# jinlong17/DA-Detect

Measured on AMD Instinct MI355X. Metric: train images/sec, DA-Faster-RCNN R-50 Cityscapes->Foggy, higher is better.
Workload: dtype f32

## Files before the change

da_detect_amd/_C.py:

```python
import contextlib
import os
import ctypes
import time

import torch

from . import _lib
from . import amax as _amax
from ._lib import ConvDesc

CL = torch.channels_last

NMS_TIE_RULE = 0

PROFILER = None
_KNAME_CACHE = {}


class KernelProfiler(object):

    def __init__(self, pool=0, only=None):
        self.only = only
        self._pool = []
        for _ in range(pool):
# ... 328 lines not shown

def _transpose_now(w, scale, wt):
    Cout, Cin, KH, KW = w.shape
    cout_pad = wt.shape[1]
    _lib.call("dadet_conv_weight_transpose_padded", _p(w), _p(scale), _p(wt), Cout, KH, KW, Cin, cout_pad, _stream())
    return wt


class _TransposeCache(object):

    def __init__(self):
        self.entries = {}
        self.epoch = 0
        self.batched_epoch = -1
        self.table = None
        self.ready = None
        self.enabled = True
        self._from_bump = False
        self._trained_only = False

    def bump(self, device=None, trained_only=False):
        self.epoch += 1
        self._trained_only = bool(trained_only)
        if self.enabled and device is not None and self.entries:
            self._from_bump = True
            try:
                self._refresh_all(device)
            finally:
                self._from_bump = False
        elif device is not None and _mode4():
            _amax.WEIGHTS.refresh(device, self.epoch, trained_only=self._trained_only)
        self._trained_only = False

    def _single(self, e, w, scale):
        _transpose_now(w, scale, e["wt"])
        _amax.WEIGHTS.invalidate(e["wt"])
        e["epoch"] = self.epoch
        if w.is_cuda:
            st = torch.cuda.current_stream(w.device)
            e["ev"] = (st, st.record_event())
        return e["wt"]

    def get(self, w, scale, cout_pad=0):
        Cout, Cin, KH, KW = w.shape
        key = (w.data_ptr(), Cout, Cin, KH, KW, scale.data_ptr() if scale is not None else 0, w.device.index, cout_pad)
        e = self.entries.get(key)
        if e is None:
            wt = torch.empty((Cin, max(Cout, cout_pad), KH, KW), dtype=torch.float32, device=w.device, memory_format=CL)
            wt._dadet_persistent = True
            e = self.entries[key] = dict(w=w, scale=scale, wt=wt, version=w._version, epoch=self.epoch, used=self.epoch,
                                         ev=None)
            self.table = None
            return self._single(e, w, scale)
        e["used"] = self.epoch
        if e["version"] != w._version:
            e["w"], e["version"] = w, w._version
            return self._single(e, w, scale)
        if e["epoch"] != self.epoch:
            if self.batched_epoch != self.epoch:
                self._refresh_all(w.device)
            if e["epoch"] != self.epoch:
                return self._single(e, w, scale)
        src = e["ev"] if e["ev"] is not None else self.ready
        if src is not None and w.is_cuda and torch.cuda.current_stream(w.device) != src[0]:
            torch.cuda.current_stream(w.device).wait_event(src[1])
        return e["wt"]
# ... 957 lines not shown
```

da_detect_amd/_lib.py:

```python
import ctypes
import os
from ctypes import POINTER, c_char_p, c_float, c_int, c_int64, c_size_t, c_uint64, c_void_p

_HERE = os.path.dirname(os.path.abspath(__file__))
LIB_PATH = os.environ.get("DADET_LIB") or os.path.join(_HERE, "libdadet_hip.so")
_lib = None
DEFAULT_GEMM_MODE = "4"


class ConvDesc(ctypes.Structure):

    _fields_ = [(n, c_int) for n in (
        "N", "H", "W", "Cin", "Cout", "KH", "KW", "stride", "pad", "Ho", "Wo", "OutH", "OutW",
        "out_spatial_stride", "relu_mode")]


class WgradPending(ctypes.Structure):

    _fields_ = [("partials", c_void_p), ("out_scale", c_void_p), ("dw", c_void_p), ("count", ctypes.c_longlong),
                ("K", c_int), ("splits", c_int), ("accumulate", c_int)]


class TransposeItem(ctypes.Structure):
    _fields_ = [("w", c_void_p), ("scale", c_void_p), ("wt", c_void_p), ("Cout", c_int), ("KH", c_int), ("KW", c_int),
                ("Cin", c_int), ("first_block", c_int), ("blocks_ci", c_int), ("blocks_co", c_int), ("cout_pad", c_int)]


class AmaxItem(ctypes.Structure):

    _fields_ = [("x", c_void_p), ("slot", c_void_p), ("n", ctypes.c_longlong), ("first_block", c_int), ("blocks", c_int)]


class MergeEntry(ctypes.Structure):

    _fields_ = [("boxes", c_void_p), ("scores", c_void_p), ("keep", c_void_p), ("count", c_void_p), ("boxes_out", c_void_p),
                ("scores_out", c_void_p), ("n", c_int), ("cap", c_int)]


class TopkRow(ctypes.Structure):

    _fields_ = [("scores", c_void_p), ("out_scores", c_void_p), ("out_idx", c_void_p), ("n", c_int), ("k", c_int)]


class SgdEntry(ctypes.Structure):

    _fields_ = [("p", c_void_p), ("g", c_void_p), ("buf", c_void_p), ("numel", c_int64),
                ("lr", c_float), ("weight_decay", c_float)]


_P = c_void_p
_SIGNATURES = {
    "dadet_version": [],
    "dadet_device_info": [POINTER(c_int), POINTER(c_int), POINTER(c_size_t), c_char_p, c_int],
    "dadet_nms_workspace_bytes": [c_int, POINTER(c_size_t)],
    "dadet_nms": [_P, _P, c_int, c_float, c_int, c_int, _P, c_size_t, _P, _P, _P],
    "dadet_roi_align_forward": [_P, _P, _P, c_int, c_int, c_int, c_int, c_int, c_int, c_int, c_float, c_int, _P],
    "dadet_roi_align_backward": [_P, _P, _P, c_int, c_int, c_int, c_int, c_int, c_int, c_int, c_float, c_int, _P],
    "dadet_roi_align_workspace_bytes": [c_int, c_int, c_int, c_int, POINTER(c_size_t)],
    "dadet_roi_align_forward_ws": [_P, _P, _P, c_int, c_int, c_int, c_int, c_int, c_int, c_int, c_float, c_int, _P, c_size_t, _P],
    "dadet_roi_align_backward_atomic": [_P, _P, _P, c_int, c_int, c_int, c_int, c_int, c_int, c_int, c_float, c_int, _P],
    "dadet_roi_align_forward_sub": [_P, _P, _P, c_int, c_int, c_int, c_int, c_int, c_int, c_int, c_float, c_int, c_int,
                                    _P, c_size_t, _P],
    "dadet_roi_align_forward_level": [_P, _P, _P, c_int, _P, c_int, c_int, c_int, c_int, c_int, c_int, c_int, c_float, c_int, _P,
                                      c_size_t, _P],
    "dadet_roi_align_backward_level": [_P, _P, _P, c_int, _P, c_int, c_int, c_int, c_int, c_int, c_int, c_int, c_float, c_int,
                                       _P],
    "dadet_roi_align_backward_sub": [_P, _P, _P, c_int, c_int, c_int, c_int, c_int, c_int, c_int, c_float, c_int, c_int,
                                     _P],
    "dadet_sigmoid_focal_loss_forward": [_P, _P, _P, c_int, c_int, c_float, c_float, _P],
    "dadet_sigmoid_focal_loss_backward": [_P, _P, _P, _P, c_int, c_int, c_float, c_float, _P],
    "dadet_conv_forward": [POINTER(ConvDesc), _P, _P, _P, _P, _P, _P, _P, _P],
    "dadet_conv_forward_scaled": [POINTER(ConvDesc), _P, _P, _P, _P, _P, _P, _P, _P, _P, _P, _P],
    "dadet_conv_wgrad_scaled": [POINTER(ConvDesc), _P, _P, c_int, _P, _P, c_int, _P, c_size_t, POINTER(WgradPending), _P, _P,
                                _P],
    "dadet_amax": [_P, ctypes.c_longlong, _P, _P],
    "dadet_amax_batch": [_P, c_int, c_int, _P],
    "dadet_conv_forward_variant": [POINTER(ConvDesc)],
    "dadet_set_gemm_mode": [c_int],
    "dadet_get_gemm_mode": [],
    "dadet_conv_wgrad_variant": [POINTER(ConvDesc)],
# ... 46 lines not shown
    "dadet_rpn_anchor_targets": [_P, _P, c_int, _P, c_int, c_float, c_float, _P, _P, _P, _P],
    "dadet_box_match_encode": [_P, c_int, _P, _P, c_int, c_float, c_float, c_float, c_float, c_float, c_float, _P, _P,
                               _P, _P],
    "dadet_roi_pool_forward": [_P, _P, _P, _P, c_int, c_int, c_int, c_int, c_int, c_int, c_int, c_float, _P],
    "dadet_roi_pool_backward": [_P, _P, _P, _P, c_int, c_int, c_int, c_int, c_int, c_int, c_int, _P],
    "dadet_deform_psroi_pool_forward": [_P, _P, _P, _P, _P, c_int, c_int, c_int, c_int, c_int, c_int, c_float,
                                        c_int, c_int, c_int, c_int, c_int, c_float, c_int, _P],
    "dadet_deform_psroi_pool_backward": [_P, _P, _P, _P, _P, _P, _P, c_int, c_int, c_int, c_int, c_int, c_int,
                                         c_float, c_int, c_int, c_int, c_int, c_int, c_float, c_int, _P],
    "dadet_relu_bn_backward": [_P, _P, _P, _P, _P, c_int64, c_int, _P],
    "dadet_relu_bn_backward_m": [_P, _P, _P, _P, _P, c_int64, c_int, _P, _P, _P],
    "dadet_colsum_workspace_bytes": [c_int64, c_int, POINTER(c_size_t)],
    "dadet_colsum": [_P, _P, c_int64, c_int, _P, c_size_t, _P],
    "dadet_colsum_ld": [_P, c_int, _P, c_int64, c_int, c_int, _P, c_size_t, _P],
    "dadet_channel_affine": [_P, _P, _P, _P, c_int64, c_int, c_int, _P],
    "dadet_maxpool3x3s2_forward": [_P, _P, c_int, c_int, c_int, c_int, c_int, c_int, _P],
    "dadet_avgpool_forward": [_P, _P, c_int, c_int, c_int, _P],
    "dadet_avgpool_backward": [_P, _P, c_int, c_int, c_int, _P],
    "dadet_nchw3_to_nhwc4": [_P, _P, c_int, c_int, c_int, _P],
    "dadet_rpn_decode_clip": [_P, _P, _P, c_int, c_float, c_float, c_float, c_float, c_float, c_float, c_float, _P, _P],
    "dadet_da_img_head_loss_forward": [_P, _P, _P, _P, _P, _P, c_int, c_int, c_int, _P],
    "dadet_da_img_head_loss_backward": [_P, _P, _P, _P, _P, _P, _P, _P, _P, c_int, c_int, c_int, _P],
    "dadet_da_img_head_loss_backward_g": [_P, _P, _P, _P, _P, _P, _P, c_float, c_float, _P, _P, _P, _P, c_int, c_int, c_int,
                                          _P],
    "dadet_da_img_head_loss_backward_gm": [_P, _P, _P, _P, _P, _P, _P, c_float, c_float, _P, _P, _P, _P, c_int, c_int, c_int,
                                          _P, _P, _P],
    "dadet_da_ins_tail_forward": [_P, _P, _P, _P, _P, _P, _P, c_int, c_int, c_int, c_int, c_int, _P],
    "dadet_da_ins_tail_backward": [_P, _P, _P, _P, _P, _P, c_float, _P, _P, _P, _P, c_int, c_int, c_int, c_int, c_int, _P],
    "dadet_da_ins_dropout_rows": [_P, _P, _P, c_int64, c_int, _P],
    "dadet_da_ins_merge": [_P, _P, _P, _P, _P, _P, c_int64, c_int, _P],
    "dadet_triplet_w_forward": [_P, _P, _P, c_int, c_int, c_int, c_float, c_float, _P, _P, _P],
    "dadet_triplet_w_backward": [_P, _P, _P, _P, _P, c_int, c_int, c_int, c_float, c_float, _P, _P, _P, _P],
    "dadet_sgd_step": [_P, c_int, c_int64, c_float, c_int, c_float, _P],
}
_RESTYPES = {"dadet_last_error": c_char_p}
EXPORTED_SYMBOLS = sorted(list(_SIGNATURES) + ["dadet_last_error"])


class DadetError(RuntimeError):
    pass


def load():
    global _lib
    if _lib is not None:
        return _lib
    if not os.path.exists(LIB_PATH):
        raise DadetError(
            "libdadet_hip.so is not built (%s). Run `python -c 'import __graft_entry__ as g; g.build()'` "
            "or `make -C da_detect_amd/csrc`. There is no CPU fallback for the product path." % LIB_PATH)
    import torch

    lib = ctypes.CDLL(LIB_PATH)
    for name, argtypes in _SIGNATURES.items():
        fn = getattr(lib, name)
        fn.argtypes = argtypes
        fn.restype = c_int
    lib.dadet_last_error.argtypes = []
    lib.dadet_last_error.restype = c_char_p
    _lib = lib
    mode = int(os.environ.get("DADET_GEMM_MODE", DEFAULT_GEMM_MODE))
    if lib.dadet_set_gemm_mode(mode) != 0:
        raise DadetError("DADET_GEMM_MODE=%d is not a valid contraction mode (0, 2, 3 or 4)" % mode)
    return lib


# ... 9 lines not shown
```

da_detect_amd/amax.py:

```python
import ctypes
import weakref

import torch

from . import _lib

STRIDE = 1 << 16
_POOL_SLOTS = STRIDE
_pools = {}
MEASURED = 0


def _stream():
    return ctypes.c_void_p(torch.cuda.current_stream().cuda_stream)


def new_slot(device):
    idx = device.index if device.index is not None else torch.cuda.current_device()
    pool = _pools.get(idx)
    if pool is None or pool[1] >= _POOL_SLOTS:
        t = torch.zeros((8, STRIDE), dtype=torch.float32, device=device)
        torch.cuda.current_stream(device).synchronize()
        pool = _pools[idx] = [t, 0]
    i = pool[1]
# ... 104 lines not shown
        if e is not None and e["ref"]() is not owner:
            d["free"].append(d["entries"].pop(key)["i"])
            d["table"] = d["table_trained"] = None
            e = None
        if e is None:
            if not d["free"]:
                self._sweep(d, epoch)
            if not d["free"]:
                raise _lib.DadetError("amax: more than %d persistent GEMM operands alive" % self.CAP)
            e = d["entries"][key] = dict(ref=weakref.ref(owner), ptr=key[0], n=key[1], i=d["free"].pop(),
                                         version=owner._version, epoch=epoch, used=epoch)
            d["table"] = d["table_trained"] = None
            self._measure_one(d, e)
        else:
            e["used"] = epoch
            if e["version"] != owner._version or e["epoch"] != epoch:
                if e["version"] == owner._version and d["epoch"] != epoch:
                    self.refresh(t.device, epoch, sync=True)
                if e["version"] != owner._version or e["epoch"] != epoch:
                    e["version"], e["epoch"] = owner._version, epoch
                    self._measure_one(d, e)
        return ctypes.c_void_p(d["slots"].data_ptr() + 4 * e["i"])

    def invalidate(self, t):
        d = self._dev(t.device)
        e = d["entries"].get((t.data_ptr(), t.numel()))
        if e is not None:
            e["epoch"] = -1

    @staticmethod
    def _frozen(e):
        o = e["ref"]()
        return isinstance(o, torch.nn.Parameter) and not o.requires_grad

    def refresh(self, device, epoch, sync=False, trained_only=False):
        if sync:
            torch.cuda.synchronize(device)
        d = self._dev(device)
        d["epoch"] = epoch
        self._sweep(d, epoch)
        live = [e for e in d["entries"].values() if self._alive(e)]
        if trained_only:
            for e in live:
                if self._frozen(e):
                    e["epoch"] = epoch
            live = [e for e in live if not self._frozen(e)]
        if not live:
            return
        keys = [(e["i"], e["ptr"], e["n"]) for e in live]
        which = "table_trained" if trained_only else "table"
        if d.get(which) is None or d[which][3] != keys:
            arr = (_lib.AmaxItem * len(live))()
            blocks = 0
            for k, e in enumerate(live):
                it = arr[k]
                n = e["n"]
                it.x, it.slot, it.n = e["ptr"], d["slots"].data_ptr() + 4 * e["i"], n
                it.first_block = blocks
                it.blocks = max(1, min(512, (n // 4 + 4095) // 4096))
                blocks += it.blocks
            host = torch.frombuffer(bytearray(bytes(arr)), dtype=torch.uint8).clone()
            idx = torch.tensor([e["i"] for e in live], dtype=torch.int64).to(device) if trained_only else None
            d[which] = (host.to(device), blocks, len(live), keys, idx)
        dev_t, blocks, n, _, idx = d[which]
        if idx is None:
            d["slots"][:, :self.CAP].zero_()
# ... 9 lines not shown
```

da_detect_amd/csrc/elementwise.hip:

```cpp
#include "box_match.h"
#include "conv_common.h"
#include <float.h>

namespace dadet {

static inline int stream_blocks(int64_t work_items, int threads) {
  int64_t b = ceil_div64(work_items, threads);
  if (b > kMaxStreamBlocks) b = kMaxStreamBlocks;
  if (b < 1) b = 1;
  return (int)b;
}

__global__ void relu_bn_backward_kernel(const float4* __restrict__ g, const float4* __restrict__ y,
                                        const float4* __restrict__ scale, float4* __restrict__ g_out,
                                        float4* __restrict__ g_scaled, int64_t total4, int C4,
                                        unsigned* __restrict__ amax_out, unsigned* __restrict__ amax_scaled) {
  float mo = 0.f, ms = 0.f;
  for (int64_t i = (int64_t)blockIdx.x * blockDim.x + threadIdx.x; i < total4;
       i += (int64_t)gridDim.x * blockDim.x) {
    const float4 gv = g[i];
    float4 r = gv;
    if (y) {
      const float4 yv = y[i];
      r.x = yv.x > 0.f ? gv.x : 0.f;
// ... 345 lines not shown
        if (!first_step) b[u] = b4[i];
      }
    }
#pragma unroll
    for (int u = 0; u < 4; ++u) {
      const int64_t i = base + u * 256 + threadIdx.x;
      if (i >= n4) continue;
      float4 d;
      d.x = g[u].x * grad_scale + wd * p[u].x; d.y = g[u].y * grad_scale + wd * p[u].y;
      d.z = g[u].z * grad_scale + wd * p[u].z; d.w = g[u].w * grad_scale + wd * p[u].w;
      float4 nb;
      if (first_step) {
        nb = d;
      } else {
        nb.x = momentum * b[u].x + d.x; nb.y = momentum * b[u].y + d.y;
        nb.z = momentum * b[u].z + d.z; nb.w = momentum * b[u].w + d.w;
      }
      b4[i] = nb;
      float4 q = p[u];
      q.x -= lr * nb.x; q.y -= lr * nb.y; q.z -= lr * nb.z; q.w -= lr * nb.w;
      p4[i] = q;
    }
  }
  for (int64_t i = n4 * 4 + (int64_t)blockIdx.x * blockDim.x + threadIdx.x; i < n;
       i += (int64_t)gridDim.x * blockDim.x) {
    float p = e.p[i];
    const float d = e.g[i] * grad_scale + wd * p;
    const float b = first_step ? d : momentum * e.buf[i] + d;
    e.buf[i] = b;
    e.p[i] = p - lr * b;
  }
}

}

using namespace dadet;

static bool aligned16(const void* p) { return (reinterpret_cast<uintptr_t>(p) & 15) == 0; }

extern "C" int dadet_relu_bn_backward(const float* g, const float* y, const float* scale, float* g_out,
                                      float* g_scaled, int64_t rows, int C, void* stream) {
  return dadet_relu_bn_backward_m(g, y, scale, g_out, g_scaled, rows, C, nullptr, nullptr, stream);
}

extern "C" int dadet_relu_bn_backward_m(const float* g, const float* y, const float* scale, float* g_out,
                                        float* g_scaled, int64_t rows, int C, float* amax_out, float* amax_scaled,
                                        void* stream) {
  DADET_REQUIRE(rows >= 0 && C > 0 && C % 4 == 0, "relu_bn_backward: C=%d must be a multiple of 4", C);
  if (rows == 0) return DADET_OK;
  DADET_REQUIRE(g && (g_out || g_scaled), "relu_bn_backward: null pointer");
  DADET_REQUIRE(aligned16(g) && aligned16(y) && aligned16(scale) && aligned16(g_out) && aligned16(g_scaled),
                "relu_bn_backward: pointers must be 16-byte aligned");
  const int64_t total4 = rows * (C / 4);
  hipLaunchKernelGGL(relu_bn_backward_kernel, dim3(stream_blocks(total4, 256)), dim3(256), 0,
                     as_stream(stream), reinterpret_cast<const float4*>(g),
                     reinterpret_cast<const float4*>(y), reinterpret_cast<const float4*>(scale),
                     reinterpret_cast<float4*>(g_out), reinterpret_cast<float4*>(g_scaled), total4, C / 4,
                     reinterpret_cast<unsigned*>(g_out ? amax_out : nullptr),
                     reinterpret_cast<unsigned*>(g_scaled ? amax_scaled : nullptr));
  return check_launch("relu_bn_backward");
}

extern "C" int dadet_colsum_workspace_bytes(int64_t rows, int C, size_t* bytes_out) {
  DADET_REQUIRE(rows >= 0 && C > 0 && bytes_out, "colsum_workspace_bytes: bad args");
  *bytes_out = rows == 0 ? 0 : sizeof(float) * (size_t)colsum_splits(rows, C) * C;
  return DADET_OK;
// ... 147 lines not shown
  DADET_REQUIRE(N >= 0 && C > 0, "focal_forward: bad dims");
  if (N == 0) return DADET_OK;
  DADET_REQUIRE(logits && targets && losses, "focal_forward: null pointer");
  const int64_t total = (int64_t)N * C;
  hipLaunchKernelGGL(focal_fwd_kernel, dim3(stream_blocks(total, 256)), dim3(256), 0, as_stream(stream),
                     logits, targets, losses, total, C, gamma, alpha);
  return check_launch("sigmoid_focal_loss_forward");
}
extern "C" int dadet_sigmoid_focal_loss_backward(const float* logits, const int32_t* targets,
                                                 const float* d_losses, float* d_logits, int N, int C,
                                                 float gamma, float alpha, void* stream) {
  DADET_REQUIRE(N >= 0 && C > 0, "focal_backward: bad dims");
  if (N == 0) return DADET_OK;
  DADET_REQUIRE(logits && targets && d_losses && d_logits, "focal_backward: null pointer");
  const int64_t total = (int64_t)N * C;
  hipLaunchKernelGGL(focal_bwd_kernel, dim3(stream_blocks(total, 256)), dim3(256), 0, as_stream(stream),
                     logits, targets, d_losses, d_logits, total, C, gamma, alpha);
  return check_launch("sigmoid_focal_loss_backward");
}

extern "C" int dadet_sgd_step(const dadet_sgd_entry* table_dev, int num_tensors, int64_t max_numel,
                              float momentum, int first_step, float grad_scale, void* stream) {
  DADET_REQUIRE(num_tensors >= 0 && max_numel >= 0, "sgd_step: bad args");
  if (num_tensors == 0 || max_numel == 0) return DADET_OK;
  DADET_REQUIRE(table_dev, "sgd_step: null table");
  DADET_REQUIRE(num_tensors <= 65535, "sgd_step: too many tensors for one launch");
  int bx = (int)ceil_div64(ceil_div64(max_numel, 4), 1024);
  if (bx > 512) bx = 512;
  if (bx < 1) bx = 1;
  hipLaunchKernelGGL(sgd_kernel, dim3(bx, num_tensors), dim3(256), 0, as_stream(stream), table_dev,
                     momentum, first_step, grad_scale);
  return check_launch("sgd_step");
}
```

da_detect_amd/solver/fused_sgd.py:

```python
import ctypes
import os

import torch

from .. import _lib
from .._lib import SgdEntry


class FusedSGD(torch.optim.Optimizer):
    def __init__(self, params, lr, momentum=0.0, weight_decay=0.0):
        defaults = dict(lr=lr, momentum=momentum, weight_decay=weight_decay)
        super(FusedSGD, self).__init__(params, defaults)
        self._table = None
        self._steps = 0
        self.reducer = None
        self.per_bucket = os.environ.get("DADET_SGD_PER_BUCKET", "1") == "1"
        self._bucket_plan = None

    def attach_reducer(self, reducer):
        self.reducer = reducer
        from ..utils import streams
        streams.enable_direct_wgrad(True)

    def zero_grad(self, set_to_none=True):
        if self.reducer is not None:
            self.reducer.zero_grad()
        else:
            super(FusedSGD, self).zero_grad(set_to_none=set_to_none)

    def _step_bucket(self, index, bucket, grad_scale):
        plan = self._bucket_table()
        if plan is None:
            return
        dev_table, ranges, device, momentum = plan
        first, n, max_numel = ranges[index]
        if n:
            _lib.call("dadet_sgd_step", ctypes.c_void_p(dev_table.data_ptr() + first * ctypes.sizeof(SgdEntry)), n,
                      ctypes.c_int64(max_numel), float(momentum), 0, float(grad_scale),
                      ctypes.c_void_p(torch.cuda.current_stream().cuda_stream))

    def _bucket_table(self):
        red = self.reducer
        order = {id(p): i for i, b in enumerate(red.buckets) for p in b["params"]}
        entries = sorted(self._entries(), key=lambda e: order.get(id(e[0]), len(red.buckets)))
        if not entries:
            self._bucket_plan = None
            return None
        momentum = entries[0][3]
        assert all(e[3] == momentum for e in entries), "FusedSGD: one momentum for all groups"
        rows, owner = [], []
        for p, lr, wd, _ in entries:
            if not p.is_cuda:
                raise _lib.DadetError("FusedSGD runs on the HIP device only")
            if id(p) not in order:
                raise _lib.DadetError("FusedSGD: a parameter outside the reducer's buckets cannot be updated bucket by bucket")
            st = self.state[p]
            if "momentum_buffer" not in st:
                st["momentum_buffer"] = torch.empty_strided(p.size(), p.stride(), dtype=p.dtype, device=p.device).zero_()
            rows.append((p.data_ptr(), p.grad.data_ptr(), st["momentum_buffer"].data_ptr(), p.numel(), lr, wd))
            owner.append(order[id(p)])
        key = tuple(rows)
        if self._bucket_plan is None or self._bucket_plan[0] != key:
            arr = (SgdEntry * len(rows))()
            for i, r in enumerate(rows):
                arr[i].p, arr[i].g, arr[i].buf, arr[i].numel, arr[i].lr, arr[i].weight_decay = r
            device = entries[0][0].device
            nbytes = ctypes.sizeof(arr)
            stage = getattr(self, "_bstage", None)
            if stage is None or stage[0][0].numel() != nbytes:
                stage = self._bstage = [(torch.empty(nbytes, dtype=torch.uint8).pin_memory(),
                                         torch.empty(nbytes, dtype=torch.uint8, device=device),
                                         torch.cuda.Event()) for _ in range(2)]
            host, dev, done = stage[self._steps % 2]
            done.synchronize()
            ctypes.memmove(host.data_ptr(), ctypes.addressof(arr), nbytes)
            dev.copy_(host, non_blocking=True)
            done.record()
            ranges = []
            for b in range(len(red.buckets)):
                idx = [i for i, o in enumerate(owner) if o == b]
                ranges.append((idx[0], len(idx), max(rows[i][3] for i in idx)) if idx else (0, 0, 0))
            self._bucket_plan = (key, dev, device, ranges, momentum)
        _, dev, device, ranges, momentum = self._bucket_plan
        return dev, ranges, device, momentum

    def _entries(self):
        out = []
        for group in self.param_groups:
            for p in group["params"]:
                if p.grad is None:
                    continue
                if self.reducer is not None and id(p) not in self._update_ids:
                    continue
                out.append((p, group["lr"], group["weight_decay"], group["momentum"]))
        return out

    @torch.no_grad()
    def step(self, closure=None, grad_scale=1.0):
        loss = None
        if closure is not None:
            with torch.enable_grad():
                loss = closure()
        handed = None
        if self.reducer is not None:
            if self.per_bucket and self.reducer.can_hand_over_buckets():
                self._update_ids = self.reducer.update_ids()
                handed = []
                self.reducer.finalize(mean=False, per_bucket=lambda i, b: handed.append(i) or self._step_bucket(
                    i, b, grad_scale / self.reducer.world_size))
            else:
                self.reducer.finalize(mean=False)
            grad_scale = grad_scale * self.reducer.mean_scale
            self._update_ids = self.reducer.update_ids()
        if handed is not None:
            self._steps += 1
            from .. import _C
            if self._bucket_plan is not None:
                _C.bump_weight_epoch(self._bucket_plan[2], trained_only=True)
            return loss
        entries = self._entries()
        if not entries:
            return loss
        momentum = entries[0][3]
        assert all(e[3] == momentum for e in entries), "FusedSGD: one momentum for all groups"
        first = []
        rows = []
        for p, lr, wd, _ in entries:
            if not p.is_cuda:
                raise _lib.DadetError("FusedSGD runs on the HIP device only")
            g = p.grad
            if g.stride() != p.stride() or not _dense(p):
                g = _like_layout(g, p)
                p.grad = g
            st = self.state[p]
            if "momentum_buffer" not in st:
                st["momentum_buffer"] = torch.empty_strided(p.size(), p.stride(), dtype=p.dtype,
                                                            device=p.device).zero_()
            first.append(False)
            rows.append((p.data_ptr(), g.data_ptr(), st["momentum_buffer"].data_ptr(), p.numel(), lr, wd))
        key = tuple(rows)
        if self._table is None or self._table[0] != key:
            arr = (SgdEntry * len(rows))()
            for i, r in enumerate(rows):
                arr[i].p, arr[i].g, arr[i].buf, arr[i].numel, arr[i].lr, arr[i].weight_decay = r
            nbytes = ctypes.sizeof(arr)
            slot = self._steps % 2
            stage = getattr(self, "_stage", None)
            if stage is None or stage[0][0].numel() != nbytes:
                device = entries[0][0].device
                stage = self._stage = [(torch.empty(nbytes, dtype=torch.uint8).pin_memory(),
                                        torch.empty(nbytes, dtype=torch.uint8, device=device),
                                        torch.cuda.Event()) for _ in range(2)]
            host, dev, done = stage[slot]
            done.synchronize()
            ctypes.memmove(host.data_ptr(), ctypes.addressof(arr), nbytes)
            dev.copy_(host, non_blocking=True)
            done.record()
            self._table = (key, dev, max(r[3] for r in rows), len(rows))
        _, dev, max_numel, n = self._table
        _lib.call("dadet_sgd_step", ctypes.c_void_p(dev.data_ptr()), n, ctypes.c_int64(max_numel),
                  float(momentum), 1 if all(first) else 0, float(grad_scale),
                  ctypes.c_void_p(torch.cuda.current_stream().cuda_stream))
        self._steps += 1
        from .. import _C
        _C.bump_weight_epoch(entries[0][0].device, trained_only=True)
        return loss


def _dense(t):
    return t.is_contiguous() or t.is_contiguous(memory_format=torch.channels_last)


def _like_layout(g, p):
    out = torch.empty_strided(p.size(), p.stride(), dtype=g.dtype, device=g.device)
    out.copy_(g)
    return out
```

include/dadet.h:

```cpp
#ifndef DADET_H_
#define DADET_H_

#include <stddef.h>
#include <stdint.h>

#ifdef __cplusplus
extern "C" {
#endif

#define DADET_OK 0
#define DADET_EINVAL (-1)
#define DADET_ELAUNCH (-2)
#define DADET_EWORKSPACE (-3)
#define DADET_EUNSUPPORTED (-4)

const char* dadet_last_error(void);
int dadet_version(void);
int dadet_device_info(int* cu_count, int* clock_khz, size_t* hbm_bytes, char* arch_name, int arch_name_len);

int dadet_nms_workspace_bytes(int n, size_t* bytes_out);
int dadet_nms(const float* boxes_xyxy, const float* scores, int n, float thresh, int tie_rule,
              int max_keep, void* workspace, size_t workspace_bytes, int64_t* keep_out,
              int* num_keep_out, void* stream);

// ... 268 lines not shown
                                      const float* g_bce, const float* g_mean_sig, const float* w_adv_dev, float w_adv,
                                      float w_cst, float* g_t_w, float* g_t_x, float* g_w2, float* g_b2, int num_images,
                                      int rows_per_image, int C1, void* stream);
int dadet_da_img_head_loss_backward_gm(const float* t, const float* w2, const float* logits, const float* labels,
                                       const float* g_bce, const float* g_mean_sig, const float* w_adv_dev, float w_adv,
                                       float w_cst, float* g_t_w, float* g_t_x, float* g_w2, float* g_b2, int num_images,
                                       int rows_per_image, int C1, float* amax_w, float* amax_x, void* stream);
int dadet_da_ins_tail_forward(const float* h, const float* w3, const float* b3, const float* labels,
                              const float* means, float* logits, float* sums, int R_bce, int R_cst, int n_src,
                              int levels, int C, void* stream);
int dadet_da_ins_tail_backward(const float* h, const float* w3, const float* logits, const float* labels,
                               const float* means, const float* coef, float inv_keep, float* g_z, float* g_w3,
                               float* g_b3, float* g_means, int R_bce, int R_cst, int n_src, int levels, int C,
                               void* stream);
int dadet_da_ins_dropout_rows(const float* h1, const float* masks, float* out, int64_t numel_per_pass, int passes,
                              void* stream);
int dadet_da_ins_merge(const float* g, const float* masks, const float* h1, const float* grl, float* g_w, float* g_x,
                       int64_t numel_per_pass, int passes, void* stream);

int dadet_triplet_w_forward(const float* anchor, const float* positive, const float* negative, int H,
                            int W, int C, float margin, float eps, float* dist_out, float* loss_sum,
                            void* stream);
int dadet_triplet_w_backward(const float* anchor, const float* positive, const float* negative,
                             const float* dist, const float* g_scale, int H, int W, int C, float margin,
                             float eps, float* g_anchor, float* g_positive, float* g_negative,
                             void* stream);

typedef struct dadet_sgd_entry {
  float* p; const float* g; float* buf; int64_t numel; float lr; float weight_decay;
} dadet_sgd_entry;
int dadet_sgd_step(const dadet_sgd_entry* table_dev, int num_tensors, int64_t max_numel, float momentum,
                   int first_step, float grad_scale, void* stream);

#ifdef __cplusplus
}
#endif
#endif
```

Before: 161.8.

## Fuse SGD update with transposed-weight refresh and amax publishing in one kernel

Adds a kernel that applies the momentum SGD update and, for conv weights with a cached transposed/flipped copy, writes the transposed (optionally scaled) weight and publishes amax values in the same pass. The optimizer builds an extended table carrying the transpose and amax-slot pointers, zeroes the claimed amax slots, then marks the transpose cache as refreshed instead of bumping the epoch and re-running separate transpose and amax kernels. This removes a second read of every updated weight and several launches per step. In exchange the host-side planning is more complex, and the fused path is tied to the weight cache bookkeeping (versions, epochs, events).

After: 162.7 (median of 6 runs). No clear change (+0.5%).

```diff
diff --git a/da_detect_amd/_C.py b/da_detect_amd/_C.py
--- a/da_detect_amd/_C.py
+++ b/da_detect_amd/_C.py
@@ -384,6 +384,33 @@
             _amax.WEIGHTS.refresh(device, self.epoch, trained_only=self._trained_only)
         self._trained_only = False
 
+    def fusable(self, device):
+        out, twice = {}, set()
+        if not self.enabled:
+            return out
+        for k, e in self.entries.items():
+            if k[6] != device.index or e["version"] != e["w"]._version:
+                continue
+            if k[0] in out:
+                twice.add(k[0])
+            out[k[0]] = (k, e)
+        for a in twice:
+            del out[a]
+        return out
+
+    def fused(self, device, done):
+        self.epoch += 1
+        for k in [k for k, e in self.entries.items() if e["used"] < self.epoch - 2]:
+            del self.entries[k]
+            self.table = None
+        for e in done:
+            e["epoch"] = self.epoch
+            e["ev"] = None
+        self.batched_epoch = self.epoch
+        if done and device.type == "cuda":
+            st = torch.cuda.current_stream(device)
+            self.ready = (st, st.record_event())
+
     def _single(self, e, w, scale):
         _transpose_now(w, scale, e["wt"])
         _amax.WEIGHTS.invalidate(e["wt"])
diff --git a/da_detect_amd/_lib.py b/da_detect_amd/_lib.py
--- a/da_detect_amd/_lib.py
+++ b/da_detect_amd/_lib.py
@@ -46,6 +46,14 @@
 
     _fields_ = [("p", c_void_p), ("g", c_void_p), ("buf", c_void_p), ("numel", c_int64),
                 ("lr", c_float), ("weight_decay", c_float)]
+
+
+class SgdRefreshEntry(ctypes.Structure):
+
+    _fields_ = [("p", c_void_p), ("g", c_void_p), ("buf", c_void_p), ("numel", c_int64),
+                ("lr", c_float), ("weight_decay", c_float), ("slot_p", c_void_p), ("wt", c_void_p), ("scale", c_void_p),
+                ("slot_wt", c_void_p), ("Cout", c_int), ("KH", c_int), ("KW", c_int), ("Cin", c_int), ("cout_pad", c_int),
+                ("reserved", c_int)]
 
 
 _P = c_void_p
@@ -158,6 +166,7 @@
     "dadet_triplet_w_forward": [_P, _P, _P, c_int, c_int, c_int, c_float, c_float, _P, _P, _P],
     "dadet_triplet_w_backward": [_P, _P, _P, _P, _P, c_int, c_int, c_int, c_float, c_float, _P, _P, _P, _P],
     "dadet_sgd_step": [_P, c_int, c_int64, c_float, c_int, c_float, _P],
+    "dadet_sgd_refresh_step": [_P, c_int, c_int, c_float, c_int, c_float, _P],
 }
 _RESTYPES = {"dadet_last_error": c_char_p}
 EXPORTED_SYMBOLS = sorted(list(_SIGNATURES) + ["dadet_last_error"])
diff --git a/da_detect_amd/amax.py b/da_detect_amd/amax.py
--- a/da_detect_amd/amax.py
+++ b/da_detect_amd/amax.py
@@ -160,6 +160,35 @@
     def _frozen(e):
         o = e["ref"]()
         return isinstance(o, torch.nn.Parameter) and not o.requires_grad
+
+    def fused_begin(self, device, epoch):
+        d = self._dev(device)
+        d["epoch"] = epoch
+        self._sweep(d, epoch)
+        out = {}
+        for k, e in d["entries"].items():
+            if not self._alive(e):
+                continue
+            if self._frozen(e):
+                e["epoch"] = epoch
+            else:
+                out[k] = e
+        return out
+
+    def slot_address(self, device, e):
+        return self._dev(device)["slots"].data_ptr() + 4 * e["i"]
+
+    def fused_zero(self, device, epoch, claimed):
+        if not claimed:
+            return
+        d = self._dev(device)
+        ids = tuple(e["i"] for e in claimed)
+        cached = d.get("fused_idx")
+        if cached is None or cached[0] != ids:
+            cached = d["fused_idx"] = (ids, torch.tensor(ids, dtype=torch.int64).to(device))
+        d["slots"].index_fill_(1, cached[1], 0.0)
+        for e in claimed:
+            e["epoch"] = epoch
 
     def refresh(self, device, epoch, sync=False, trained_only=False):
         if sync:
diff --git a/da_detect_amd/csrc/elementwise.hip b/da_detect_amd/csrc/elementwise.hip
--- a/da_detect_amd/csrc/elementwise.hip
+++ b/da_detect_amd/csrc/elementwise.hip
@@ -401,6 +401,172 @@
   }
 }
 
+__device__ __forceinline__ float sgd_update(float p, float g, float& b, float lr, float wd, float momentum,
+                                            int first_step, float grad_scale) {
+  const float d = g * grad_scale + wd * p;
+  const float nb = first_step ? d : momentum * b + d;
+  b = nb;
+  return p - lr * nb;
+}
+__device__ __forceinline__ float amax4(float m, const float4& v) {
+  return fmaxf(fmaxf(m, fmaxf(fabsf(v.x), fabsf(v.y))), fmaxf(fabsf(v.z), fabsf(v.w)));
+}
+
+constexpr int kRefreshTiles = 4;
+
+__global__ __launch_bounds__(256) void sgd_refresh_kernel(const dadet_sgd_refresh_entry* __restrict__ table,
+                                                          float momentum, int first_step, float grad_scale) {
+  __shared__ float tile[kRefreshTiles][32][33];
+  const dadet_sgd_refresh_entry e = table[blockIdx.y];
+  const float lr = e.lr, wd = e.weight_decay;
+  unsigned* slot_p = reinterpret_cast<unsigned*>(e.slot_p);
+  float mp = 0.f;
+  if (!e.wt) {
+    const int64_t n = e.numel;
+    const bool vec = ((reinterpret_cast<uintptr_t>(e.p) | reinterpret_cast<uintptr_t>(e.g) |
+                       reinterpret_cast<uintptr_t>(e.buf)) & 15) == 0;
+    const int64_t n4 = vec ? n / 4 : 0;
+    if ((int64_t)blockIdx.x * 1024 >= n4 && ((int64_t)blockIdx.x * 256 >= n - n4 * 4)) return;
+    float4* p4 = reinterpret_cast<float4*>(e.p);
+    const float4* g4 = reinterpret_cast<const float4*>(e.g);
+    float4* b4 = reinterpret_cast<float4*>(e.buf);
+    for (int64_t base = (int64_t)blockIdx.x * 1024; base < n4; base += (int64_t)gridDim.x * 1024) {
+      float4 p[4], g[4], b[4];
+#pragma unroll
+      for (int u = 0; u < 4; ++u) {
+        const int64_t i = base + u * 256 + threadIdx.x;
+        if (i < n4) {
+          p[u] = p4[i];
+          g[u] = g4[i];
+          if (!first_step) b[u] = b4[i];
+        }
+      }
+#pragma unroll
+      for (int u = 0; u < 4; ++u) {
+        const int64_t i = base + u * 256 + threadIdx.x;
+        if (i >= n4) continue;
+        float4 q;
+        q.x = sgd_update(p[u].x, g[u].x, b[u].x, lr, wd, momentum, first_step, grad_scale);
+        q.y = sgd_update(p[u].y, g[u].y, b[u].y, lr, wd, momentum, first_step, grad_scale);
+        q.z = sgd_update(p[u].z, g[u].z, b[u].z, lr, wd, momentum, first_step, grad_scale);
+        q.w = sgd_update(p[u].w, g[u].w, b[u].w, lr, wd, momentum, first_step, grad_scale);
+        b4[i] = b[u];
+        p4[i] = q;
+        mp = amax4(mp, q);
+      }
+    }
+    for (int64_t i = n4 * 4 + (int64_t)blockIdx.x * blockDim.x + threadIdx.x; i < n;
+         i += (int64_t)gridDim.x * blockDim.x) {
+      float b = first_step ? 0.f : e.buf[i];
+      const float q = sgd_update(e.p[i], e.g[i], b, lr, wd, momentum, first_step, grad_scale);
+      e.buf[i] = b;
+      e.p[i] = q;
+      mp = fmaxf(mp, fabsf(q));
+    }
+    if (slot_p) amax_publish(slot_p, mp);
+    return;
+  }
+  const int Cout = e.Cout, Cin = e.Cin, taps = e.KH * e.KW;
+  const int cout_pad = e.cout_pad > Cout ? e.cout_pad : Cout;
+  const int blocks_ci = (Cin + 31) >> 5, blocks_co = (cout_pad + 31) >> 5;
+  const int tiles = blocks_ci * blocks_co * taps;
+  if ((int)blockIdx.x * kRefreshTiles >= tiles) return;
+  const int64_t K = (int64_t)taps * Cin, Kt = (int64_t)taps * cout_pad;
+  const bool vec = (Cin & 3) == 0 && ((reinterpret_cast<uintptr_t>(e.p) | reinterpret_cast<uintptr_t>(e.g) |
+                                       reinterpret_cast<uintptr_t>(e.buf)) & 15) == 0;
+  const int lj = threadIdx.x >> 3, lc = (threadIdx.x & 7) * 4;
+  const int tx = threadIdx.x & 31, ty = threadIdx.x >> 5;
+  float mt = 0.f;
+  for (int t0 = (int)blockIdx.x * kRefreshTiles; t0 < tiles; t0 += (int)gridDim.x * kRefreshTiles) {
+    float p[kRefreshTiles][4], g[kRefreshTiles][4], b[kRefreshTiles][4];
+#pragma unroll
+    for (int u = 0; u < kRefreshTiles; ++u) {
+      const int t = t0 + u;
+      const int bx = t % blocks_ci, by = (t / blocks_ci) % blocks_co, tap = t / (blocks_ci * blocks_co);
+      const int co = by * 32 + lj, ci = bx * 32 + lc;
+      const int64_t off = (int64_t)co * K + (int64_t)tap * Cin + ci;
+#pragma unroll
+      for (int k = 0; k < 4; ++k) p[u][k] = g[u][k] = b[u][k] = 0.f;
+      if (t < tiles && co < Cout) {
+        if (vec) {
+          if (ci < Cin) {
+            const float4 pv = *reinterpret_cast<const float4*>(e.p + off);
+            const float4 gv = *reinterpret_cast<const float4*>(e.g + off);
+            p[u][0] = pv.x; p[u][1] = pv.y; p[u][2] = pv.z; p[u][3] = pv.w;
+            g[u][0] = gv.x; g[u][1] = gv.y; g[u][2] = gv.z; g[u][3] = gv.w;
+            if (!first_step) {
+              const float4 bv = *reinterpret_cast<const float4*>(e.buf + off);
+              b[u][0] = bv.x; b[u][1] = bv.y; b[u][2] = bv.z; b[u][3] = bv.w;
+            }
+          }
+        } else {
+#pragma unroll
+          for (int k = 0; k < 4; ++k)
+            if (ci + k < Cin) {
+              p[u][k] = e.p[off + k];
+              g[u][k] = e.g[off + k];
+              if (!first_step) b[u][k] = e.buf[off + k];
+            }
+        }
+      }
+    }
+#pragma unroll
+    for (int u = 0; u < kRefreshTiles; ++u) {
+      const int t = t0 + u;
+      const int bx = t % blocks_ci, by = (t / blocks_ci) % blocks_co, tap = t / (blocks_ci * blocks_co);
+      const int co = by * 32 + lj, ci = bx * 32 + lc;
+      const int64_t off = (int64_t)co * K + (int64_t)tap * Cin + ci;
+      const bool row = t < tiles && co < Cout;
+      float q[4];
+#pragma unroll
+      for (int k = 0; k < 4; ++k) {
+        const bool in = row && ci + k < Cin;
+        q[k] = in ? sgd_update(p[u][k], g[u][k], b[u][k], lr, wd, momentum, first_step, grad_scale) : 0.f;
+        if (in) mp = fmaxf(mp, fabsf(q[k]));
+      }
+      if (row) {
+        if (vec) {
+          if (ci < Cin) {
+            *reinterpret_cast<float4*>(e.buf + off) = make_float4(b[u][0], b[u][1], b[u][2], b[u][3]);
+            *reinterpret_cast<float4*>(e.p + off) = make_float4(q[0], q[1], q[2], q[3]);
+          }
+        } else {
+#pragma unroll
+          for (int k = 0; k < 4; ++k)
+            if (ci + k < Cin) {
+              e.buf[off + k] = b[u][k];
+              e.p[off + k] = q[k];
+            }
+        }
+      }
+      const float sc = (e.scale && row) ? e.scale[co] : 1.f;
+#pragma unroll
+      for (int k = 0; k < 4; ++k) {
+        float v = q[k];
+        if (e.scale && row && ci + k < Cin) v = v * sc;
+        tile[u][lj][lc + k] = v;
+        mt = fmaxf(mt, fabsf(v));
+      }
+    }
+    __syncthreads();
+#pragma unroll
+    for (int u = 0; u < kRefreshTiles; ++u) {
+      const int t = t0 + u;
+      if (t >= tiles) break;
+      const int bx = t % blocks_ci, by = (t / blocks_ci) % blocks_co, tap = t / (blocks_ci * blocks_co);
+      const int r = tap / e.KW, sidx = tap % e.KW;
+      const int tapT = (e.KH - 1 - r) * e.KW + (e.KW - 1 - sidx);
+      for (int j = ty; j < 32; j += 8) {
+        const int ci = bx * 32 + j, co = by * 32 + tx;
+        if (co < cout_pad && ci < Cin) e.wt[(int64_t)ci * Kt + (int64_t)tapT * cout_pad + co] = tile[u][tx][j];
+      }
+    }
+    __syncthreads();
+  }
+  if (slot_p) amax_publish(slot_p, mp);
+  if (e.slot_wt) amax_publish(reinterpret_cast<unsigned*>(e.slot_wt), mt);
+}
+
 }
 
 using namespace dadet;
@@ -614,3 +780,15 @@
                      momentum, first_step, grad_scale);
   return check_launch("sgd_step");
 }
+
+extern "C" int dadet_sgd_refresh_step(const dadet_sgd_refresh_entry* table_dev, int num_tensors, int max_units,
+                                      float momentum, int first_step, float grad_scale, void* stream) {
+  DADET_REQUIRE(num_tensors >= 0 && max_units >= 0, "sgd_refresh_step: bad args");
+  if (num_tensors == 0 || max_units == 0) return DADET_OK;
+  DADET_REQUIRE(table_dev, "sgd_refresh_step: null table");
+  DADET_REQUIRE(num_tensors <= 65535, "sgd_refresh_step: too many tensors for one launch");
+  const int bx = max_units > 512 ? 512 : max_units;
+  hipLaunchKernelGGL(sgd_refresh_kernel, dim3(bx, num_tensors), dim3(256), 0, as_stream(stream), table_dev,
+                     momentum, first_step, grad_scale);
+  return check_launch("sgd_refresh_step");
+}
diff --git a/da_detect_amd/solver/fused_sgd.py b/da_detect_amd/solver/fused_sgd.py
--- a/da_detect_amd/solver/fused_sgd.py
+++ b/da_detect_amd/solver/fused_sgd.py
@@ -4,7 +4,8 @@
 import torch
 
 from .. import _lib
-from .._lib import SgdEntry
+from .. import amax as _amax
+from .._lib import SgdEntry, SgdRefreshEntry
 
 
 class FusedSGD(torch.optim.Optimizer):
@@ -16,6 +17,7 @@
         self.reducer = None
         self.per_bucket = os.environ.get("DADET_SGD_PER_BUCKET", "1") == "1"
         self._bucket_plan = None
+        self._bucket_step = None
 
     def attach_reducer(self, reducer):
         self.reducer = reducer
@@ -29,60 +31,126 @@
             super(FusedSGD, self).zero_grad(set_to_none=set_to_none)
 
     def _step_bucket(self, index, bucket, grad_scale):
-        plan = self._bucket_table()
+        plan = self._bucket_step
         if plan is None:
             return
-        dev_table, ranges, device, momentum = plan
-        first, n, max_numel = ranges[index]
+        if plan["fused"] and not plan["zeroed"]:
+            _amax.WEIGHTS.fused_zero(plan["device"], plan["epoch"], plan["claimed"])
+            plan["zeroed"] = True
+        first, n, size = plan["ranges"][index]
         if n:
-            _lib.call("dadet_sgd_step", ctypes.c_void_p(dev_table.data_ptr() + first * ctypes.sizeof(SgdEntry)), n,
-                      ctypes.c_int64(max_numel), float(momentum), 0, float(grad_scale),
-                      ctypes.c_void_p(torch.cuda.current_stream().cuda_stream))
-
-    def _bucket_table(self):
+            self._launch(plan["dev"].data_ptr() + first * ctypes.sizeof(plan["row_type"]), n, size, plan["momentum"], 0,
+                         grad_scale, plan["fused"])
+
+    def _launch(self, table_ptr, n, size, momentum, first_step, grad_scale, fused):
+        if fused:
+            _lib.call("dadet_sgd_refresh_step", ctypes.c_void_p(table_ptr), n, int(size), float(momentum), first_step,
+                      float(grad_scale), ctypes.c_void_p(torch.cuda.current_stream().cuda_stream))
+        else:
+            _lib.call("dadet_sgd_step", ctypes.c_void_p(table_ptr), n, ctypes.c_int64(size), float(momentum), first_step,
+                      float(grad_scale), ctypes.c_void_p(torch.cuda.current_stream().cuda_stream))
+
+    def _rows(self, entries, relayout):
+        rows = []
+        for p, lr, wd, _ in entries:
+            if not p.is_cuda:
+                raise _lib.DadetError("FusedSGD runs on the HIP device only")
+            g = p.grad
+            if g.stride() != p.stride() or not _dense(p):
+                if not relayout:
+                    raise _lib.DadetError("FusedSGD: gradient of a %s parameter (strides %s) with strides %s cannot be "
+                                          "updated bucket by bucket" % (tuple(p.shape), p.stride(), g.stride()))
+                g = _like_layout(g, p)
+                p.grad = g
+            st = self.state[p]
+            if "momentum_buffer" not in st:
+                st["momentum_buffer"] = torch.empty_strided(p.size(), p.stride(), dtype=p.dtype,
+                                                            device=p.device).zero_()
+            rows.append((p.data_ptr(), g.data_ptr(), st["momentum_buffer"].data_ptr(), p.numel(), lr, wd))
+        return rows
+
+    def _refresh_columns(self, entries, rows, device):
+        from .. import _C
+        epoch = _C._TRANSPOSES.epoch + 1
+        forms = _C._TRANSPOSES.fusable(device)
+        slots = _amax.WEIGHTS.fused_begin(device, epoch) if _C._mode4() else {}
+        ext, units, done, claimed = [], [], [], []
+
+        def slot(ptr, n):
+            e = slots.get((ptr, n))
+            if e is None:
+                return 0
+            claimed.append(e)
+            return _amax.WEIGHTS.slot_address(device, e)
+
+        for (p, _, _, _), r in zip(entries, rows):
+            sp = slot(r[0], r[3])
+            f = forms.get(r[0])
+            if f is not None and f[0][1] * f[0][2] * f[0][3] * f[0][4] == r[3] and p.dim() == 4 \
+                    and p.is_contiguous(memory_format=torch.channels_last):
+                (_, Cout, Cin, KH, KW, _, _, cout_pad), e = f
+                wt, sc = e["wt"], e["scale"]
+                ext.append((sp, wt.data_ptr(), sc.data_ptr() if sc is not None else 0, slot(wt.data_ptr(), wt.numel()),
+                            Cout, KH, KW, Cin, cout_pad))
+                units.append((((Cin + 31) // 32) * ((max(Cout, cout_pad) + 31) // 32) * KH * KW + 3) // 4)
+                done.append(e)
+            else:
+                ext.append((sp, 0, 0, 0, 0, 0, 0, 0, 0))
+                units.append(max(1, (r[3] + 4095) // 4096))
+        return ext, units, done, claimed, epoch
+
+    def _upload(self, which, row_type, rows, device):
+        arr = (row_type * len(rows))()
+        names = [f[0] for f in row_type._fields_]
+        for i, r in enumerate(rows):
+            it = arr[i]
+            for k, v in zip(names, r):
+                setattr(it, k, v)
+        nbytes = ctypes.sizeof(arr)
+        stage = getattr(self, which, None)
+        if stage is None or stage[0][0].numel() != nbytes:
+            stage = [(torch.empty(nbytes, dtype=torch.uint8).pin_memory(),
+                      torch.empty(nbytes, dtype=torch.uint8, device=device), torch.cuda.Event()) for _ in range(2)]
+            setattr(self, which, stage)
+        host, dev, done = stage[self._steps % 2]
+        done.synchronize()
+        ctypes.memmove(host.data_ptr(), ctypes.addressof(arr), nbytes)
+        dev.copy_(host, non_blocking=True)
+        done.record()
+        return dev
+
+    def _bucket_table(self, fused):
         red = self.reducer
         order = {id(p): i for i, b in enumerate(red.buckets) for p in b["params"]}
         entries = sorted(self._entries(), key=lambda e: order.get(id(e[0]), len(red.buckets)))
         if not entries:
-            self._bucket_plan = None
-            return None
+            self._bucket_plan = self._bucket_step = None
+            return
         momentum = entries[0][3]
         assert all(e[3] == momentum for e in entries), "FusedSGD: one momentum for all groups"
-        rows, owner = [], []
-        for p, lr, wd, _ in entries:
-            if not p.is_cuda:
-                raise _lib.DadetError("FusedSGD runs on the HIP device only")
+        for p, _, _, _ in entries:
             if id(p) not in order:
                 raise _lib.DadetError("FusedSGD: a parameter outside the reducer's buckets cannot be updated bucket by bucket")
-            st = self.state[p]
-            if "momentum_buffer" not in st:
-                st["momentum_buffer"] = torch.empty_strided(p.size(), p.stride(), dtype=p.dtype, device=p.device).zero_()
-            rows.append((p.data_ptr(), p.grad.data_ptr(), st["momentum_buffer"].data_ptr(), p.numel(), lr, wd))
-            owner.append(order[id(p)])
-        key = tuple(rows)
+        rows = self._rows(entries, relayout=False)
+        owner = [order[id(e[0])] for e in entries]
+        device = entries[0][0].device
+        plan = dict(fused=fused, device=device, momentum=momentum, zeroed=False, done=[], claimed=[], epoch=None,
+                    row_type=SgdRefreshEntry if fused else SgdEntry)
+        if fused:
+            ext, size, plan["done"], plan["claimed"], plan["epoch"] = self._refresh_columns(entries, rows, device)
+            rows = [r + x for r, x in zip(rows, ext)]
+        else:
+            size = [r[3] for r in rows]
+        key = (fused, tuple(rows))
         if self._bucket_plan is None or self._bucket_plan[0] != key:
-            arr = (SgdEntry * len(rows))()
-            for i, r in enumerate(rows):
-                arr[i].p, arr[i].g, arr[i].buf, arr[i].numel, arr[i].lr, arr[i].weight_decay = r
-            device = entries[0][0].device
-            nbytes = ctypes.sizeof(arr)
-            stage = getattr(self, "_bstage", None)
-            if stage is None or stage[0][0].numel() != nbytes:
-                stage = self._bstage = [(torch.empty(nbytes, dtype=torch.uint8).pin_memory(),
-                                         torch.empty(nbytes, dtype=torch.uint8, device=device),
-                                         torch.cuda.Event()) for _ in range(2)]
-            host, dev, done = stage[self._steps % 2]
-            done.synchronize()
-            ctypes.memmove(host.data_ptr(), ctypes.addressof(arr), nbytes)
-            dev.copy_(host, non_blocking=True)
-            done.record()
+            dev = self._upload("_bstage", plan["row_type"], rows, device)
             ranges = []
             for b in range(len(red.buckets)):
                 idx = [i for i, o in enumerate(owner) if o == b]
-                ranges.append((idx[0], len(idx), max(rows[i][3] for i in idx)) if idx else (0, 0, 0))
+                ranges.append((idx[0], len(idx), max(size[i] for i in idx)) if idx else (0, 0, 0))
             self._bucket_plan = (key, dev, device, ranges, momentum)
-        _, dev, device, ranges, momentum = self._bucket_plan
-        return dev, ranges, device, momentum
+        plan["dev"], plan["ranges"] = self._bucket_plan[1], self._bucket_plan[3]
+        self._bucket_step = plan
 
     def _entries(self):
         out = []
@@ -101,10 +169,13 @@
         if closure is not None:
             with torch.enable_grad():
                 loss = closure()
+        from .. import _C
+        fused = os.environ.get("DADET_SGD_FUSED_REFRESH", "1") == "1"
         handed = None
         if self.reducer is not None:
             if self.per_bucket and self.reducer.can_hand_over_buckets():
                 self._update_ids = self.reducer.update_ids()
+                self._bucket_table(fused)
                 handed = []
                 self.reducer.finalize(mean=False, per_bucket=lambda i, b: handed.append(i) or self._step_bucket(
                     i, b, grad_scale / self.reducer.world_size))
@@ -114,56 +185,39 @@
             self._update_ids = self.reducer.update_ids()
         if handed is not None:
             self._steps += 1
-            from .. import _C
-            if self._bucket_plan is not None:
-                _C.bump_weight_epoch(self._bucket_plan[2], trained_only=True)
+            plan = self._bucket_step
+            if plan is not None:
+                if plan["fused"] and handed:
+                    _C._TRANSPOSES.fused(plan["device"], plan["done"])
+                else:
+                    _C.bump_weight_epoch(plan["device"], trained_only=True)
             return loss
         entries = self._entries()
         if not entries:
             return loss
         momentum = entries[0][3]
         assert all(e[3] == momentum for e in entries), "FusedSGD: one momentum for all groups"
-        first = []
-        rows = []
-        for p, lr, wd, _ in entries:
-            if not p.is_cuda:
-                raise _lib.DadetError("FusedSGD runs on the HIP device only")
-            g = p.grad
-            if g.stride() != p.stride() or not _dense(p):
-                g = _like_layout(g, p)
-                p.grad = g
-            st = self.state[p]
-            if "momentum_buffer" not in st:
-                st["momentum_buffer"] = torch.empty_strided(p.size(), p.stride(), dtype=p.dtype,
-                                                            device=p.device).zero_()
-            first.append(False)
-            rows.append((p.data_ptr(), g.data_ptr(), st["momentum_buffer"].data_ptr(), p.numel(), lr, wd))
-        key = tuple(rows)
+        rows = self._rows(entries, relayout=True)
+        device = entries[0][0].device
+        done = claimed = epoch = None
+        if fused:
+            ext, size, done, claimed, epoch = self._refresh_columns(entries, rows, device)
+            rows = [r + x for r, x in zip(rows, ext)]
+        else:
+            size = [r[3] for r in rows]
+        key = (fused, tuple(rows))
         if self._table is None or self._table[0] != key:
-            arr = (SgdEntry * len(rows))()
-            for i, r in enumerate(rows):
-                arr[i].p, arr[i].g, arr[i].buf, arr[i].numel, arr[i].lr, arr[i].weight_decay = r
-            nbytes = ctypes.sizeof(arr)
-            slot = self._steps % 2
-            stage = getattr(self, "_stage", None)
-            if stage is None or stage[0][0].numel() != nbytes:
-                device = entries[0][0].device
-                stage = self._stage = [(torch.empty(nbytes, dtype=torch.uint8).pin_memory(),
-                                        torch.empty(nbytes, dtype=torch.uint8, device=device),
-                                        torch.cuda.Event()) for _ in range(2)]
-            host, dev, done = stage[slot]
-            done.synchronize()
-            ctypes.memmove(host.data_ptr(), ctypes.addressof(arr), nbytes)
-            dev.copy_(host, non_blocking=True)
-            done.record()
-            self._table = (key, dev, max(r[3] for r in rows), len(rows))
-        _, dev, max_numel, n = self._table
-        _lib.call("dadet_sgd_step", ctypes.c_void_p(dev.data_ptr()), n, ctypes.c_int64(max_numel),
-                  float(momentum), 1 if all(first) else 0, float(grad_scale),
-                  ctypes.c_void_p(torch.cuda.current_stream().cuda_stream))
+            dev = self._upload("_stage", SgdRefreshEntry if fused else SgdEntry, rows, device)
+            self._table = (key, dev, max(size), len(rows))
+        _, dev, size, n = self._table
+        if fused:
+            _amax.WEIGHTS.fused_zero(device, epoch, claimed)
+        self._launch(dev.data_ptr(), n, size, momentum, 0, grad_scale, fused)
         self._steps += 1
-        from .. import _C
-        _C.bump_weight_epoch(entries[0][0].device, trained_only=True)
+        if fused:
+            _C._TRANSPOSES.fused(device, done)
+        else:
+            _C.bump_weight_epoch(device, trained_only=True)
         return loss
 
 
diff --git a/include/dadet.h b/include/dadet.h
--- a/include/dadet.h
+++ b/include/dadet.h
@@ -324,6 +324,15 @@
 int dadet_sgd_step(const dadet_sgd_entry* table_dev, int num_tensors, int64_t max_numel, float momentum,
                    int first_step, float grad_scale, void* stream);
 
+typedef struct dadet_sgd_refresh_entry {
+  float* p; const float* g; float* buf; int64_t numel; float lr; float weight_decay;
+  float* slot_p;
+  float* wt; const float* scale; float* slot_wt;
+  int Cout, KH, KW, Cin, cout_pad, reserved;
+} dadet_sgd_refresh_entry;
+int dadet_sgd_refresh_step(const dadet_sgd_refresh_entry* table_dev, int num_tensors, int max_units, float momentum,
+                           int first_step, float grad_scale, void* stream);
+
 #ifdef __cplusplus
 }
 #endif
```
